# DaehwanKimLab/hisat-genotype

Hardware: NVIDIA B200
Metric: reads typed/sec (higher is better)
Workload: dtype u64 bitsets + f64 EM

## Files before the change

hisat-genotype_b200/csrc/em.cu:

```cuda
#include <cooperative_groups.h>
#include <math.h>
#include <string.h>

#include <algorithm>
#include <vector>

#include "common.cuh"

namespace cg = cooperative_groups;

namespace {

constexpr int EM_THREADS = 1024;
constexpr int EM_WARPS = EM_THREADS / 32;
constexpr int MODE_INIT = 0, MODE_NEXT = 1, MODE_FIRSTK = 2;
constexpr int32_t FK_NONE = 0x7fffffff;

__device__ unsigned long long g_em_trace[16];
__device__ int g_em_trace_on;
struct Trace {
    bool on;
    long long t;
    unsigned long long ns0;
    __device__ __forceinline__ void start() {
        on = g_em_trace_on && blockIdx.x == 0 && threadIdx.x == 0;
        t = on ? clock64() : 0;
        ns0 = 0;
        if (g_em_trace_on && threadIdx.x == 0) asm volatile("mov.u64 %0, %%globaltimer;" : "=l"(ns0));
    }
    __device__ __forceinline__ void finish() {
        if (g_em_trace_on && threadIdx.x == 0) {
            unsigned long long ns1;
            asm volatile("mov.u64 %0, %%globaltimer;" : "=l"(ns1));
            atomicAdd(&g_em_trace[11], ns1 - ns0);
            atomicMax(&g_em_trace[12], ns1 - ns0);
            atomicAdd(&g_em_trace[13], 1ull);
        }
    }
    __device__ __forceinline__ void mark(int k) {
        if (on) {
            const long long n = clock64();
            atomicAdd(&g_em_trace[k], (unsigned long long)(n - t));
            t = n;
        }
    }
    __device__ __forceinline__ void count(int k) {
        if (on) atomicAdd(&g_em_trace[k], 1ull);
    }
};

constexpr int EM_PEER_MAX = 16, EM_PEER_G = 256;
constexpr unsigned long long EM_PEER_TIMEOUT_NS = 4000000000ull;
constexpr size_t EM_PEER_FLAG_BYTES = (size_t)EM_PEER_MAX * EM_PEER_G * 4, EM_PEER_HDR = EM_PEER_FLAG_BYTES + 256;
struct EmPeer {
    int rank, world;
    unsigned char *block[EM_PEER_MAX];
};
__device__ __forceinline__ void st_release_sys(uint32_t *p, uint32_t v) {
    asm volatile("st.release.sys.global.u32 [%0], %1;" ::"l"(p), "r"(v) : "memory");
}
__device__ __forceinline__ uint32_t ld_acquire_sys(const uint32_t *p) {
    uint32_t v;
    asm volatile("ld.acquire.sys.global.u32 %0, [%1];" : "=r"(v) : "l"(p) : "memory");
    return v;
}
__device__ __forceinline__ double ld_sys_f64(const double *p) {
    double v;
    asm volatile("ld.relaxed.sys.global.f64 %0, [%1];" : "=d"(v) : "l"(p) : "memory");
    return v;
}
__device__ __forceinline__ int32_t ld_sys_s32(const int32_t *p) {
    int32_t v;
    asm volatile("ld.relaxed.sys.global.s32 %0, [%1];" : "=r"(v) : "l"(p) : "memory");
    return v;
}

struct EmArgs {
    const uint64_t *bits;
    const double *cnt;
    const double *len;
    int C, A, wp, remove_low, fixed_iters;
    int slab_rows;
    int compact;
    int A_live_max;
    unsigned slab_bytes;
    uint64_t *dense_ws;
    uint64_t *mv_ws;
    int32_t *rep_ws;
    double *mult_ws;
    const unsigned long long *cnt_u64;
    const int32_t *C_ptr;
    const int32_t *class_first;
    int32_t key_offset;
    const EmPeer *peer;
    double *prob;
    uint8_t *in_result;
    int32_t *first_class;
    int32_t *iters_status;
    double *vec;
    uint8_t *live;
    double *part_acc;
    int32_t *part_aux;
    double *red_acc;
    int32_t *red_aux;
};

struct Smem {
    uint64_t *mbar;
    double *red;
    double *p;
    double *w;
    uint8_t *valid;
    uint64_t *slab;
    const int32_t *lv;
    double *cnt;
    uint64_t *cm64;
    unsigned char *c64;
    const int32_t *row_off;
    const int32_t *col_off;
// ... 595 lines not shown
                    }
                    v3[j] = x;
                }
            }
            if (lane == 0) s_flag = flag;
        }
        __syncthreads();
        const int flag = s_flag;
        if (flag == 2) {
            if (tid == 0) *status = HGT_ERR_KEY;
            __syncthreads();
            break;
        }
        if (flag == 1) {
            compact_sweep(a, c, v3, l2, v1, l1, status);
            sweeps += 1;
            last = 3;
        } else {
            last = 0;
        }
        have_last = true;
        if (warp == 0) {
            double d = 0.0;
            for (int j = lane; j < c.n; j += 32)
                if (l0[j]) d += l1[j] ? fabs(v0[j] - v1[j]) : v0[j];
            d = warp_sum(d);
            if (lane == 0) s_diff = d;
        }
        __syncthreads();
        diff = s_diff;
        if (tid < 64) {
            const double t = v0[tid];
            const int tl = l0[tid];
            v0[tid] = v1[tid];
            l0[tid] = l1[tid];
            v1[tid] = t;
            l1[tid] = tl;
        }
        __syncthreads();
        if (last == 0) last = 1;
        if (iter >= 10 && a.remove_low) {
            if (warp == 0) {
                double mx = -1.0;
                for (int j = lane; j < c.n; j += 32)
                    if (l0[j]) mx = fmax(mx, v0[j]);
                mx = warp_max(mx);
                if (mx >= 0.0) {
                    const double thr = mx / 10.0;
                    for (int j = lane; j < c.n; j += 32)
                        if (l0[j] && !(v0[j] >= thr)) {
                            l0[j] = 0;
                            v0[j] = 0.0;
                        }
                }
            }
            __syncthreads();
        }
        iter++;
    }
}

constexpr int DEDUP_CAP = 8192;
constexpr int DEDUP_MAX_LIVE = 6144;
constexpr int DEDUP_COLS = 4;
__host__ __device__ inline bool em_merge_fits(int wp, int A_live_max, size_t slab_bytes) {
    return wp <= DEDUP_COLS * EM_WARPS && A_live_max <= DEDUP_MAX_LIVE && slab_bytes >= (size_t)wp * 64 * 12 + DEDUP_CAP * 4 &&
           slab_bytes >= (size_t)wp * 8 * 32;
}
__host__ __device__ inline bool em_collapse_fits(bool compacted, int C, int wp, int slab_rows) {
    return compacted || (size_t)C * 24 + 64 * 64 <= p_slots((size_t)wp * 64) * 8 + (size_t)slab_rows * 8 + (size_t)slab_rows * wp * 8;
}
__device__ __forceinline__ unsigned long long dedup_mix(unsigned long long x) {
    x ^= x >> 33; x *= 0xff51afd7ed558ccdULL; x ^= x >> 33; x *= 0xc4ceb9fe1a85ec53ULL; x ^= x >> 33;
    return x;
}

__device__ int em_compact_build(const EmArgs &a, Smem &sm, int32_t *lv, int C, int *s_int, bool dedup, Trace &tr) {
    const int tid = threadIdx.x, lane = tid & 31, warp = tid >> 5;
    const int wp = a.wp;
    uint64_t *lw = reinterpret_cast<uint64_t *>(sm.c64);
    int32_t *base = reinterpret_cast<int32_t *>(sm.c64 + 2048);
    for (int j = tid; j < 256; j += EM_THREADS) lw[j] = 0ull;
    __syncthreads();
    {
        uint64_t acc[8];
#pragma unroll
        for (int i = 0; i < 8; i++) acc[i] = 0ull;
        for (int r = warp; r < C; r += EM_WARPS) {
            const uint64_t *row = a.bits + (size_t)r * wp;
#pragma unroll
            for (int i = 0; i < 8; i++) {
                const int j = lane + 32 * i;
                if (j < wp) acc[i] |= row[j];
            }
        }
#pragma unroll
        for (int i = 0; i < 8; i++)
            if (acc[i]) atomicOr(reinterpret_cast<unsigned long long *>(&lw[lane + 32 * i]), (unsigned long long)acc[i]);
    }
    __syncthreads();
    tr.mark(5);
    if (dedup) {
        int32_t *cnt32 = reinterpret_cast<int32_t *>(a.dense_ws);
        const int Atot = wp * 64;
        for (int al = tid; al < Atot; al += EM_THREADS) { cnt32[al] = 0; a.rep_ws[al] = -1; }
        unsigned long long *xs = reinterpret_cast<unsigned long long *>(sm.w);
        uint32_t *ys = reinterpret_cast<uint32_t *>(sm.cnt);
        for (int r = tid; r < C; r += EM_THREADS) {
            const unsigned long long x = dedup_mix((unsigned long long)r + 1ull);
            xs[r] = x;
            ys[r] = (uint32_t)dedup_mix(x ^ 0x9e3779b97f4a7c15ull);
        }
        uint64_t *tile = sm.slab;
        const int T = min(C, (int)(a.slab_bytes / ((size_t)wp * 8)));
        uint64_t pa[DEDUP_COLS], pb[DEDUP_COLS], pc[DEDUP_COLS];
#pragma unroll
        for (int c = 0; c < DEDUP_COLS; c++) pa[c] = pb[c] = pc[c] = 0ull;
        for (int t0 = 0; t0 < C; t0 += T) {
            const int nr = min(T, C - t0);
            __syncthreads();
            {
                const ulonglong2 *src = reinterpret_cast<const ulonglong2 *>(a.bits + (size_t)t0 * wp);
                ulonglong2 *dst = reinterpret_cast<ulonglong2 *>(tile);
                const int n2 = nr * wp / 2;
#pragma unroll 4
                for (int i = tid; i < n2; i += EM_THREADS) dst[i] = __ldg(&src[i]);
            }
            __syncthreads();
            const int j0 = warp * DEDUP_COLS;
            if (j0 < wp) {
                const bool v1 = j0 + 1 < wp, v2 = j0 + 2 < wp, v3 = j0 + 3 < wp;
                for (int r = 0; r < nr; r++) {
                    const ulonglong2 *trow = reinterpret_cast<const ulonglong2 *>(tile + (size_t)r * wp + j0);
                    const ulonglong2 q01 = trow[0], q23 = trow[1];
                    const uint64_t w0 = q01.x, w1 = v1 ? q01.y : 0ull, w2 = v2 ? q23.x : 0ull, w3 = v3 ? q23.y : 0ull;
                    if ((w0 | w1 | w2 | w3) == 0ull) continue;
                    const unsigned long long x = xs[t0 + r];
                    const uint32_t y = ys[t0 + r];
                    const uint64_t m0 = ((x >> lane) & 1ull) ? ~0ull : 0ull, m1 = ((x >> (lane + 32)) & 1ull) ? ~0ull : 0ull,
                                   m2 = ((y >> lane) & 1u) ? ~0ull : 0ull;
                    pa[0] ^= w0 & m0; pb[0] ^= w0 & m1; pc[0] ^= w0 & m2;
                    pa[1] ^= w1 & m0; pb[1] ^= w1 & m1; pc[1] ^= w1 & m2;
                    pa[2] ^= w2 & m0; pb[2] ^= w2 & m1; pc[2] ^= w2 & m2;
                    pa[3] ^= w3 & m0; pb[3] ^= w3 & m1; pc[3] ^= w3 & m2;
                }
            }
        }
        __syncthreads();
        tr.mark(14);
        unsigned long long *sig1 = reinterpret_cast<unsigned long long *>(sm.slab);
        uint32_t *sig2 = reinterpret_cast<uint32_t *>(sig1 + Atot);
#pragma unroll
        for (int c = 0; c < DEDUP_COLS; c++) {
            const int j = warp * DEDUP_COLS + c;
            if (j >= wp) continue;
            const uint64_t live = lw[j];
            for (int b = 0; b < 64; b++) {
                if (!((live >> b) & 1ull)) continue;
                const unsigned m0 = __ballot_sync(0xffffffffu, (pa[c] >> b) & 1ull);
                const unsigned m1 = __ballot_sync(0xffffffffu, (pb[c] >> b) & 1ull);
                const unsigned m2 = __ballot_sync(0xffffffffu, (pc[c] >> b) & 1ull);
                if (lane == 0) {
                    sig1[j * 64 + b] = (unsigned long long)m0 | ((unsigned long long)m1 << 32);
                    sig2[j * 64 + b] = m2;
                }
            }
        }
        __syncthreads();
        uint32_t *occ = sig2 + Atot;
        for (int i = tid; i < DEDUP_CAP; i += EM_THREADS) occ[i] = 0xffffffffu;
        __syncthreads();
        for (int al = tid; al < Atot; al += EM_THREADS) {
            if (!((lw[al >> 6] >> (al & 63)) & 1ull)) continue;
            const unsigned long long h1 = sig1[al];
            const uint32_t h2 = sig2[al];
            unsigned slot = (unsigned)dedup_mix(h1 + h2) & (DEDUP_CAP - 1);
            while (true) {
                const uint32_t prev = atomicCAS(&occ[slot], 0xffffffffu, ((uint32_t)al << 16) | (uint32_t)al);
                if (prev == 0xffffffffu) break;
                const int owner = (int)(prev >> 16);
                if (sig1[owner] == h1 && sig2[owner] == h2) {
                    atomicMin(&occ[slot], ((uint32_t)owner << 16) | (uint32_t)al);
                    break;
                }
                slot = (slot + 1) & (DEDUP_CAP - 1);
            }
            a.rep_ws[al] = (int)slot;
        }
        __syncthreads();
        for (int al = tid; al < Atot; al += EM_THREADS) {
            const int slot = a.rep_ws[al];
            if (slot < 0) continue;
            const int rp = (int)(occ[slot] & 0xffffu);
            a.rep_ws[al] = rp;
            if (rp != al) atomicAdd(&cnt32[rp], 1);
        }
        __syncthreads();
        for (int al = tid; al < Atot; al += EM_THREADS) {
            const int rp = a.rep_ws[al];
            if (rp >= 0 && rp != al) atomicAnd(reinterpret_cast<unsigned long long *>(&lw[al >> 6]), ~(1ull << (al & 63)));
        }
        __syncthreads();
        tr.mark(15);
    }
    if (warp == 0) {
        int run = 0;
        for (int j0 = 0; j0 < wp; j0 += 32) {
            const int j = j0 + lane;
            const int c = j < wp ? __popcll(lw[j]) : 0;
            int incl = c;
#pragma unroll
            for (int o = 1; o < 32; o <<= 1) {
                const int y = __shfl_up_sync(0xffffffffu, incl, o);
                if (lane >= o) incl += y;
            }
            if (j < wp) base[j] = run + incl - c;
            run += __shfl_sync(0xffffffffu, incl, 31);
        }
        if (lane == 0) *s_int = run;
    }
    __syncthreads();
    const int An = *s_int;
    if (An > a.A_live_max) return An;
    for (int j = tid; j < wp; j += EM_THREADS) {
        uint64_t m = lw[j];
        int n = base[j];
        while (m) {
            const int b = __ffsll((long long)m) - 1;
            m &= m - 1;
            lv[n++] = j * 64 + b;
// ... 89 lines not shown
            if (r < C) row_off[r + 1] = run + incl;
            run += __shfl_sync(0xffffffffu, incl, 31);
        }
        if (lane == 0) row_off[0] = 0;
    }
    for (int c = tid; c < wq; c += EM_THREADS) {
        int n = 0;
        for (int w = 0; w < nb; w++) {
            nzpre[(size_t)c * nb + w] = (uint32_t)n;
            n += __popc(nzbits[(size_t)c * nb + w]);
        }
        col_off[c + 1] = n;
    }
    __syncthreads();
    if (warp == 0) {
        int run = 0;
        for (int c0 = 0; c0 < wq; c0 += 32) {
            const int c = c0 + lane;
            const int v = c < wq ? col_off[c + 1] : 0;
            int incl = v;
#pragma unroll
            for (int o = 1; o < 32; o <<= 1) {
                const int y = __shfl_up_sync(0xffffffffu, incl, o);
                if (lane >= o) incl += y;
            }
            if (c < wq) col_off[c + 1] = run + incl;
            run += __shfl_sync(0xffffffffu, incl, 31);
        }
        if (lane == 0) col_off[0] = 0;
    }
    __syncthreads();
    const int nnzw = row_off[C];
    const size_t need = ((fixed + 15) & ~(size_t)15) + (size_t)nnzw * 16 + 32;
    if (need > R_bytes || C > 65535) {
        __syncthreads();
        for (int i = tid; i < C * wpc; i += EM_THREADS) sm.slab[i] = __ldcg(&dense[i]);
        __syncthreads();
        return An;
    }
    uint64_t *r_ent = reinterpret_cast<uint64_t *>(R + ((fixed + 15) & ~(size_t)15));
    uint64_t *c_ent = r_ent + ((nnzw + 1) & ~1);
    for (int r = warp; r < C; r += EM_WARPS) {
        int pos = row_off[r];
        for (int c0 = 0; c0 < wq; c0 += 32) {
            const int c = c0 + lane;
            const uint32_t word = c < wq ? __ldcg(&dense32[(size_t)r * wq + c]) : 0u;
            const unsigned nzm = __ballot_sync(0xffffffffu, word != 0u);
            if (word != 0u) {
                const int e = pos + __popc(nzm & ((1u << lane) - 1u));
                r_ent[e] = (uint64_t)word | ((uint64_t)((uint32_t)c * 264u) << 32);
                const int ce = col_off[c] + (int)nzpre[(size_t)c * nb + (r >> 5)] +
                               __popc(nzbits[(size_t)c * nb + (r >> 5)] & ((1u << (r & 31)) - 1u));
                c_ent[ce] = (uint64_t)word | ((uint64_t)((uint32_t)r * 8u) << 32);
            }
            pos += __popc(nzm);
        }
    }
    __syncthreads();
    sm.row_off = row_off; sm.col_off = col_off;
    sm.r_ent = r_ent; sm.c_ent = c_ent;
    return An;
}

template <int NA, bool COOP>
__global__ void __launch_bounds__(EM_THREADS, 1) em_kernel(const EmArgs *__restrict__ args_arr) {
    extern __shared__ __align__(16) unsigned char smem_raw[];
    EmArgs a = COOP ? args_arr[0] : args_arr[blockIdx.x];
    if (a.C_ptr) a.C = min(*a.C_ptr, a.C);
    const int tid = threadIdx.x;
    const int A_orig = a.A;
    __shared__ int s_status;
    __shared__ int s_int;
    if (tid == 0) s_status = HGT_OK;
    Trace tr, tr_all;
    tr.start();
    tr_all = tr;
    tr.count(10);
    Smem sm;
    sm.mbar = reinterpret_cast<uint64_t *>(smem_raw);
    sm.red = reinterpret_cast<double *>(smem_raw + 16);
    sm.lv = nullptr; sm.cnt = nullptr; sm.cm64 = nullptr; sm.c64 = nullptr;
    sm.row_off = nullptr; sm.col_off = nullptr; sm.r_ent = nullptr; sm.c_ent = nullptr; sm.dense_g = nullptr;
    sm.mult = nullptr;
    bool compacted = false;
    if (!COOP && a.compact) {
        const int wpc_max = max(2, ((a.A_live_max + 63) / 64 + 1) & ~1);
        const size_t Apadc = (size_t)wpc_max * 64, Cpad = (size_t)a.slab_rows;
        unsigned char *q = smem_raw + 16 + 40 * 8;
        sm.c64 = q; q += 4096;
        int32_t *lv = reinterpret_cast<int32_t *>(q); q += Apadc * 4;
        sm.p = reinterpret_cast<double *>(q); q += p_slots(Apadc) * 8;
        sm.w = reinterpret_cast<double *>(q); q += Cpad * 8;
        sm.cnt = reinterpret_cast<double *>(q); q += Cpad * 8;
        sm.cm64 = reinterpret_cast<uint64_t *>(q); q += Cpad * 8;
        sm.slab = reinterpret_cast<uint64_t *>(q); q += a.slab_bytes;
        sm.valid = q;
        for (int al = tid; al < A_orig; al += EM_THREADS) {
            a.prob[al] = 0.0;
            a.in_result[al] = 0;
            a.first_class[al] = FK_NONE;
        }
        const bool dedup = !a.len && a.rep_ws && em_merge_fits(a.wp, a.A_live_max, a.slab_bytes);
        const int An = em_compact_build(a, sm, lv, a.C, &s_int, dedup, tr);
        if (An > a.A_live_max) {
            if (tid == 0) {
                a.iters_status[0] = 0;
                a.iters_status[1] = HGT_ERR_ARG;
                a.iters_status[2] = 0;
            }
            return;
        }
        sm.lv = lv;
        a.A = An;
        a.wp = max(2, ((An + 63) / 64 + 1) & ~1);
        compacted = true;
    } else {
        const int Apad0 = a.wp * 64;
        sm.p = sm.red + 40;
        sm.w = sm.p + p_slots(Apad0);
        sm.slab = reinterpret_cast<uint64_t *>(sm.w + a.slab_rows);
        sm.valid = reinterpret_cast<uint8_t *>(sm.slab + (size_t)a.slab_rows * a.wp);
    }
    const int Apad = a.wp * 64;
    if (tid == 0) {
        mbar_init(sm.mbar, 1);
        fence_barrier_init();
    }
    __syncthreads();
    int row_lo = 0, row_hi = a.C;
    if (COOP) {
        const int G = gridDim.x;
        const int per = (a.C + G - 1) / G;
        row_lo = min(a.C, (int)blockIdx.x * per);
        row_hi = min(a.C, row_lo + per);
    }
    const bool resident = compacted || (row_hi - row_lo) <= a.slab_rows;
    bool loaded = compacted;
    uint32_t parity = 0;
    uint32_t xseq = 0;
    if (COOP && a.peer) xseq = *reinterpret_cast<const volatile uint32_t *>(a.peer->block[a.peer->rank] + EM_PEER_FLAG_BYTES + 4);
    double *v0 = a.vec, *v1 = a.vec + Apad, *v2 = a.vec + 2 * (size_t)Apad, *v3 = a.vec + 3 * (size_t)Apad;
    uint8_t *l0 = a.live, *l1 = a.live + Apad, *l2 = a.live + 2 * (size_t)Apad;
    tr.mark(5);
    em_sweep<NA, COOP>(a, sm, MODE_INIT, nullptr, nullptr, v0, l0, nullptr, row_lo, row_hi, resident, loaded,
                       parity, &s_status, tr, xseq);
    double diff = 1.0;
    int iter = 0, sweeps = 0;
    const double *last_in = v0;
    const uint8_t *last_live = l0;
    bool have_last = false;
    const bool compact_ok = !COOP && em_collapse_fits(compacted, a.C, a.wp, a.slab_rows);
    while (a.fixed_iters > 0 ? iter < a.fixed_iters : (diff > 0.0001 && iter < 1000)) {
        if (s_status != HGT_OK) break;
        if (compact_ok && (iter == 0 || (iter > 10 && a.remove_low))) {
            int cnt_live = 0;
            for (int al = tid; al < a.A; al += EM_THREADS)
                if (l0[al]) cnt_live += (sm.mult && sm.mult[al] != 1.0) ? 1000 : 1;
            cnt_live = (int)block_sum((double)cnt_live, sm.red);
            if (cnt_live > 0 && cnt_live <= 64) {
                Compact c;
                unsigned char *base = compacted ? sm.c64 : reinterpret_cast<unsigned char *>(sm.p);
                c.v = reinterpret_cast<double *>(base);
                c.len = c.v + 256;
                c.q = c.len + 64;
                c.lv = reinterpret_cast<int *>(c.q + 64);
                c.l = c.lv + 64;
                if (compacted) {
                    c.cnt = sm.cnt;
                    c.w = sm.w;
                    c.cm = sm.cm64;
                } else {
                    c.cnt = reinterpret_cast<double *>(c.l + 192);
                    c.w = c.cnt + a.C;
                    c.cm = reinterpret_cast<uint64_t *>(c.w + a.C);
                }
                c.n = cnt_live;
                __syncthreads();
                if (tid < 32) {
                    int n = 0;
                    for (int a0 = 0; a0 < a.A; a0 += 32) {
                        const int al = a0 + tid;
                        const bool k = al < a.A && l0[al];
                        const unsigned m = __ballot_sync(0xffffffffu, k);
                        if (k) c.lv[n + __popc(m & ((1u << tid) - 1u))] = al;
                        n += __popc(m);
                    }
                }
                __syncthreads();
                if (tid < 64) {
                    const bool k = tid < c.n;
                    const int al = k ? c.lv[tid] : 0;
                    c.v[tid] = k ? v0[al] : 0.0;
                    c.v[64 + tid] = c.v[128 + tid] = c.v[192 + tid] = 0.0;
                    c.l[tid] = k ? 1 : 0;
                    c.l[64 + tid] = c.l[128 + tid] = 0;
                    c.len[tid] = (k && a.len) ? a.len[orig_allele(sm, al)] : 1.0;
                }
                {
                    const int lane = tid & 31, warp = tid >> 5;
                    const int a_lo = lane < c.n ? c.lv[lane] : -1, a_hi = lane + 32 < c.n ? c.lv[lane + 32] : -1;
                    for (int r = warp; r < a.C; r += EM_WARPS) {
                        const uint64_t *row = (compacted ? sm.dense_g : a.bits) + (size_t)r * a.wp;
                        const bool b_lo = a_lo >= 0 && ((__ldcg(&row[a_lo >> 6]) >> (a_lo & 63)) & 1ull);
                        const bool b_hi = a_hi >= 0 && ((__ldcg(&row[a_hi >> 6]) >> (a_hi & 63)) & 1ull);
                        const unsigned m_lo = __ballot_sync(0xffffffffu, b_lo), m_hi = __ballot_sync(0xffffffffu, b_hi);
                        if (lane == 0) {
                            c.cm[r] = (uint64_t)m_lo | ((uint64_t)m_hi << 32);
                            if (!compacted) c.cnt[r] = a.cnt_u64 ? (double)a.cnt_u64[r] : a.cnt[r];
                        }
                    }
                }
// ... 58 lines not shown
            __syncthreads();
            break;
        }
        if (ssv > 0.0) {
            const double g = -sqrt(ssr / ssv);
            for (int al = tid; al < a.A; al += EM_THREADS) {
                double x = 0.0;
                if (l0[al]) {
                    const double r = v1[al] - v0[al];
                    const double v = v2[al] - v1[al] - r;
                    x = v0[al] - 2 * g * r + g * g * v;
                    x = x > 0.0 ? x : 0.0;
                }
                v3[al] = x;
            }
            __syncthreads();
            tr.mark(6);
            em_sweep<NA, COOP>(a, sm, MODE_NEXT, v3, l2, v1, l1, nullptr, row_lo, row_hi, resident, loaded,
                               parity, &s_status, tr, xseq);
            sweeps += 1;
            last_in = v3;
            last_live = l2;
        } else {
            last_in = v0;
            last_live = l0;
        }
        have_last = true;
        double d = 0.0;
        for (int al = tid; al < a.A; al += EM_THREADS)
            if (l0[al]) d += l1[al] ? fabs(v0[al] - v1[al]) : v0[al];
        diff = block_sum(d, sm.red);
        {
            double *tv = v0; v0 = v1; v1 = tv;
            uint8_t *tl = l0; l0 = l1; l1 = tl;
        }
        if (iter >= 10 && a.remove_low) {
            em_prune(a, sm, v0, l0);
        }
        iter++;
    }
    if (s_status == HGT_OK) {
        if (a.remove_low) em_prune(a, sm, v0, l0);
        double part = 0.0;
        int nk = 0;
        for (int al = tid; al < a.A; al += EM_THREADS)
            if (l0[al]) {
                part += a.len ? v0[al] / a.len[orig_allele(sm, al)] : v0[al];
                nk = 1;
            }
        const double total = block_sum(part, sm.red);
        if (block_or(nk) && !(total > 0.0) && !(total < 0.0)) {
            if (tid == 0) s_status = HGT_ERR_ZERODIV;
            __syncthreads();
        }
        const bool writer = !COOP || blockIdx.x == 0;
        if (writer) {
            for (int al = tid; al < a.A; al += EM_THREADS) {
                const bool key = l0[al];
                const int ao = orig_allele(sm, al);
                a.prob[ao] = key ? (a.len ? v0[al] / a.len[ao] / total : (sm.mult ? v0[al] / sm.mult[al] / total : v0[al] / total)) : 0.0;
                a.in_result[ao] = key ? 1 : 0;
            }
        }
        if (have_last) {
            em_sweep<NA, COOP>(a, sm, MODE_FIRSTK, last_in, last_live, nullptr, nullptr, a.first_class, row_lo,
                               row_hi, resident, loaded, parity, &s_status, tr, xseq);
        } else if (writer) {
            for (int al = tid; al < A_orig; al += EM_THREADS) a.first_class[al] = FK_NONE;
        }
        if (sm.mult) {
            __syncthreads();
            for (int al = tid; al < A_orig; al += EM_THREADS) {
                const int rp = a.rep_ws[al];
                if (rp >= 0 && rp != al) {
                    a.prob[al] = a.prob[rp];
                    a.in_result[al] = a.in_result[rp];
                    a.first_class[al] = a.first_class[rp];
                }
            }
        }
    }
    tr.mark(6);
    tr_all.mark(8);
    tr_all.finish();
    if (tid == 0 && (!COOP || blockIdx.x == 0)) {
        a.iters_status[0] = iter;
        a.iters_status[1] = s_status;
        a.iters_status[2] = sweeps;
        if (COOP && a.peer) *reinterpret_cast<uint32_t *>(a.peer->block[a.peer->rank] + EM_PEER_FLAG_BYTES + 4) = xseq;
    }
}

template <int NA>
__global__ void __launch_bounds__(EM_THREADS, 1) em_part_kernel(EmArgs a, int mode, const double *__restrict__ pin) {
    extern __shared__ __align__(16) unsigned char smem_raw[];
    const int tid = threadIdx.x;
    Smem sm;
    sm.mbar = reinterpret_cast<uint64_t *>(smem_raw);
    sm.red = reinterpret_cast<double *>(smem_raw + 16);
    sm.lv = nullptr; sm.cnt = nullptr; sm.cm64 = nullptr; sm.c64 = nullptr;
    sm.row_off = nullptr; sm.col_off = nullptr; sm.r_ent = nullptr; sm.c_ent = nullptr; sm.dense_g = nullptr;
    sm.mult = nullptr;
    const int Apad = a.wp * 64;
    sm.p = sm.red + 40;
    sm.w = sm.p + p_slots(Apad);
    sm.slab = reinterpret_cast<uint64_t *>(sm.w + a.slab_rows);
    sm.valid = reinterpret_cast<uint8_t *>(sm.slab + (size_t)a.slab_rows * a.wp);
    if (tid == 0) {
        mbar_init(sm.mbar, 1);
        fence_barrier_init();
    }
    __syncthreads();
    const int G = gridDim.x, g = blockIdx.x;
    const int per = (a.C + G - 1) / G;
    const int row_lo = min(a.C, g * per), row_hi = min(a.C, row_lo + per);
    bool loaded = false;
    uint32_t parity = 0;
    double acc[NA];
    int32_t fk[NA];
    uint32_t hit = 0;
    Trace tr;
    tr.on = false; tr.t = 0; tr.ns0 = 0;
    em_accumulate<NA>(a, sm, mode, pin, nullptr, row_lo, row_hi, false, loaded, parity, acc, fk, hit, tr);
#pragma unroll
    for (int i = 0; i < NA; i++) {
        const int al = tid + i * EM_THREADS;
        if (al < a.A) {
            a.part_acc[(size_t)g * Apad + al] = acc[i];
            a.part_aux[(size_t)g * Apad + al] = (mode == MODE_FIRSTK) ? fk[i] : (int32_t)((hit >> i) & 1u);
        }
    }
}

__global__ void em_part_reduce_kernel(int G, int A, int Apad, int mode, const double *__restrict__ part_acc,
                                      const int32_t *__restrict__ part_aux, double *__restrict__ acc_out,
                                      int32_t *__restrict__ aux_out, double *__restrict__ hit_out) {
    const int al = blockIdx.x * blockDim.x + threadIdx.x;
    if (al >= A) return;
    double s = 0.0;
    int32_t x = (mode == MODE_FIRSTK) ? FK_NONE : 0;
    for (int g = 0; g < G; g++) {
        s += part_acc[(size_t)g * Apad + al];
        const int32_t y = part_aux[(size_t)g * Apad + al];
        x = (mode == MODE_FIRSTK) ? min(x, y) : (x | y);
    }
    if (acc_out) acc_out[al] = s;
    if (aux_out) aux_out[al] = x;
    if (hit_out) hit_out[al] = (double)x;
}

struct EmPlan {
    int na;
    int slab_rows;
    size_t smem;
};

int em_plan(const hgt_ctx *ctx, int rows_per_cta, int A, int wp, EmPlan *plan) {
    const int Apad = wp * 64;
    if (A > 16 * EM_THREADS) {
        hgt_set_error("EM kernel supports at most %d alleles per problem (got %d)", 16 * EM_THREADS, A);
        return HGT_ERR_UNSUPPORTED;
    }
    int na = 1;
    while (na * EM_THREADS < Apad) na *= 2;
    const size_t fixed = 16 + 40 * 8 + p_slots(Apad) * 8;
    const size_t budget = ctx->smem_optin > 1024 ? ctx->smem_optin - 1024 : 0;
    if (fixed + 2 * ((size_t)wp * 8 + 9) > budget) {
        hgt_set_error("EM kernel: %d alleles do not fit shared memory", A);
        return HGT_ERR_UNSUPPORTED;
    }
    size_t rows = (budget - fixed) / ((size_t)wp * 8 + 9);
    rows &= ~(size_t)1;
    int want = rows_per_cta < 2 ? 2 : ((rows_per_cta + 1) & ~1);
    if ((size_t)want < rows) rows = want;
    plan->na = na;
    plan->slab_rows = (int)rows;
    plan->smem = fixed + rows * ((size_t)wp * 8 + 8) + rows + 16;
    return HGT_OK;
}

template <bool COOP>
int em_launch(hgt_ctx *ctx, cudaStream_t st, const EmArgs *d_args, int grid, int na, size_t smem) {
    void (*kern)(const EmArgs *) = nullptr;
    switch (na) {
        case 1: kern = em_kernel<1, COOP>; break;
        case 2: kern = em_kernel<2, COOP>; break;
        case 4: kern = em_kernel<4, COOP>; break;
        case 8: kern = em_kernel<8, COOP>; break;
        default: kern = em_kernel<16, COOP>; break;
    }
    HGT_CUDA(hgt_smem_at_least((const void *)kern, smem));
    if (COOP) {
        void *params[] = {(void *)&d_args};
        HGT_CUDA(cudaLaunchCooperativeKernel((void *)kern, dim3(grid), dim3(EM_THREADS), params, smem, st));
    } else {
        kern<<<grid, EM_THREADS, smem, st>>>(d_args);
        HGT_CUDA(cudaGetLastError());
    }
    ctx->launches++;
    return HGT_OK;
}

constexpr size_t EM_DENSE_SCRATCH = 232448;
struct EmShape {
    int C, A, wp, A_live_max;
};
int em_plan_batched(const hgt_ctx *ctx, const EmShape &sh, EmArgs *a, int *na, size_t *smem) {
    const size_t budget = ctx->smem_optin > 1024 ? ctx->smem_optin - 1024 : 0;
    int alive = sh.A_live_max < sh.A ? sh.A_live_max : sh.A;
    if (alive < 1) alive = 1;
    const int wpc = hgt_row_pitch(alive);
    const size_t Apadc = (size_t)wpc * 64;
    const size_t Cpad = sh.C < 2 ? 2 : (size_t)((sh.C + 1) & ~1);
    const size_t dense = Cpad * (size_t)wpc * 8;
    const size_t other = 16 + 40 * 8 + 4096 + Apadc * 4 + p_slots(Apadc) * 8 + Cpad * 25 + 16;
    size_t need = other + dense;
    if (sh.wp <= 256 && need <= budget && dense <= EM_DENSE_SCRATCH && Apadc <= (size_t)16 * EM_THREADS) {
        const size_t nb = (Cpad + 31) / 32;
        size_t want = 4 * dense + (Cpad + 1 + 2 * (size_t)wpc + 1 + 4 * (size_t)wpc * nb) * 4 + 64;
        want = (want + 15) & ~(size_t)15;
        size_t slab = dense;
        if (other + want <= budget) slab = want;
        else if (budget - other > dense) slab = (budget - other) & ~(size_t)15;
        need = other + slab;
        a->slab_bytes = (unsigned)slab;
        a->compact = 1;
        a->A_live_max = alive;
        a->slab_rows = (int)Cpad;
        int n = 1;
        while ((size_t)n * EM_THREADS < Apadc) n *= 2;
        *na = n;
        *smem = need;
        return HGT_OK;
    }
    EmPlan plan;
    HGT_CHECK(em_plan(ctx, sh.C < 1 ? 1 : sh.C, sh.A, sh.wp, &plan));
    a->compact = 0;
    a->slab_bytes = 0;
    a->A_live_max = sh.A;
    a->slab_rows = plan.slab_rows;
    *na = plan.na;
    *smem = plan.smem;
    return HGT_OK;
}

int em_launch_batched(hgt_ctx *ctx, cudaStream_t st, int n, const EmArgs *planned, const int *na, const size_t *smem,
                      EmArgs *h_args, EmArgs *d_args, bool h_pinned) {
    std::vector<int> order(n);
    for (int i = 0; i < n; i++) order[i] = i;
    std::stable_sort(order.begin(), order.end(), [&](int x, int y) {
        if (planned[x].compact != planned[y].compact) return planned[x].compact < planned[y].compact;
        return (double)planned[x].C * planned[x].A_live_max > (double)planned[y].C * planned[y].A_live_max;
    });
    for (int i = 0; i < n; i++) h_args[i] = planned[order[i]];
    if (h_pinned) HGT_CUDA(hgt_small_h2d(d_args, h_args, (size_t)n * sizeof(EmArgs), st));
    else HGT_CUDA(cudaMemcpyAsync(d_args, h_args, (size_t)n * sizeof(EmArgs), cudaMemcpyHostToDevice, st));
    int na_max = 1;
    size_t sm = 0;
    for (int i = 0; i < n; i++) {
        if (na[i] > na_max) na_max = na[i];
        if (smem[i] > sm) sm = smem[i];
    }
    HGT_CHECK(em_launch<false>(ctx, st, d_args, n, na_max, sm));
    return HGT_OK;
}

inline size_t align_up(size_t x, size_t a) { return (x + a - 1) / a * a; }
inline size_t em_compact_scratch_bytes(int wp) { return align_up(EM_DENSE_SCRATCH + (size_t)wp * 48 + (size_t)wp * 64 * 12, 256); }
inline void em_set_scratch(EmArgs *a, void *scratch) {
    unsigned char *b = static_cast<unsigned char *>(scratch);
    a->dense_ws = reinterpret_cast<uint64_t *>(b);
    a->mv_ws = reinterpret_cast<uint64_t *>(b + EM_DENSE_SCRATCH);
    a->mult_ws = reinterpret_cast<double *>(b + EM_DENSE_SCRATCH + (size_t)a->wp * 48);
    a->rep_ws = reinterpret_cast<int32_t *>(b + EM_DENSE_SCRATCH + (size_t)a->wp * 48 + (size_t)a->wp * 64 * 8);
}

struct EmWs {
    EmArgs *d_args;
    double *vec;
    uint8_t *live;
    double *part_acc;
    int32_t *part_aux;
    double *red_acc;
    int32_t *red_aux;
    void *scratch;
};
size_t em_ws_bytes(int sm_count, int A) {
    const size_t Apad = (size_t)hgt_row_pitch(A) * 64;
    size_t b = 512;
    b += align_up(4 * Apad * 8, 256);
    b += align_up(4 * Apad, 256);
    b += align_up((size_t)sm_count * Apad * 8, 256);
    b += align_up((size_t)sm_count * Apad * 4, 256);
    b += align_up(Apad * 8, 256) + align_up(Apad * 4, 256);
    b += em_compact_scratch_bytes(hgt_row_pitch(A));
    return b;
}
EmWs em_ws_carve(void *ws, int sm_count, int A) {
    const size_t Apad = (size_t)hgt_row_pitch(A) * 64;
    unsigned char *p = static_cast<unsigned char *>(ws);
    EmWs w;
    w.d_args = reinterpret_cast<EmArgs *>(p); p += 512;
    w.vec = reinterpret_cast<double *>(p); p += align_up(4 * Apad * 8, 256);
    w.live = p; p += align_up(4 * Apad, 256);
    w.part_acc = reinterpret_cast<double *>(p); p += align_up((size_t)sm_count * Apad * 8, 256);
    w.part_aux = reinterpret_cast<int32_t *>(p); p += align_up((size_t)sm_count * Apad * 4, 256);
    w.red_acc = reinterpret_cast<double *>(p); p += align_up(Apad * 8, 256);
    w.red_aux = reinterpret_cast<int32_t *>(p); p += align_up(Apad * 4, 256);
    w.scratch = p;
    return w;
}

int em_dev_plan(const hgt_ctx *ctx, int n_classes, int n_alleles, int wp, int n_ctas, int A_live_max, EmArgs *a,
                EmPlan *plan, int *grid) {
    int G = n_ctas;
    if (G <= 0) {
        const size_t bytes = (size_t)n_classes * wp * 8;
        G = bytes <= 160 * 1024 ? 1 : ctx->sm_count;
    }
    if (G > ctx->sm_count) G = ctx->sm_count;
    if (G > n_classes) G = n_classes;
    if (G < 1) G = 1;
    if (G == 1) {
        const EmShape sh{n_classes, n_alleles, wp, A_live_max};
        int na = 1;
        size_t smem = 0;
        HGT_CHECK(em_plan_batched(ctx, sh, a, &na, &smem));
        plan->na = na; plan->smem = smem; plan->slab_rows = a->slab_rows;
    } else {
        HGT_CHECK(em_plan(ctx, (n_classes + G - 1) / G, n_alleles, wp, plan));
        a->compact = 0; a->A_live_max = n_alleles; a->slab_bytes = 0;
        a->slab_rows = plan->slab_rows;
    }
    *grid = G;
    return HGT_OK;
// ... 462 lines not shown
        for (int al = tid; al < A; al += EM_THREADS) {
            const double a0 = p0[al], an = pn[al];
            const uint8_t k0 = l0[al], kn = ln[al];
            if (k0) d += kn ? fabs(a0 - an) : a0;
            lastp[al] = use3 ? (l2[al] ? p3[al] : 0.0) : (k0 ? a0 : 0.0);
            lastl[al] = use3 ? l2[al] : k0;
            p0[al] = an;
            l0[al] = kn;
        }
        d = block_sum(d, red);
        if (it >= 10 && remove_low) shard_prune(A, p0, l0, red);
        if (tid == 0) s.scal[4] = d;
    } else {
        double *p0 = s.vec, *prob = s.vec + A;
        uint8_t *l0 = s.live;
        if (remove_low) shard_prune(A, p0, l0, red);
        double part = 0.0;
        int any = 0;
        for (int al = tid; al < A; al += EM_THREADS)
            if (l0[al]) {
                part += len ? p0[al] / len[al] : p0[al];
                any = 1;
            }
        const double total = block_sum(part, red);
        any = block_or(any);
        if (any && !(total > 0.0) && !(total < 0.0) && tid == 0) s.scal[3] = 1.0;
        for (int al = tid; al < A; al += EM_THREADS)
            prob[al] = l0[al] ? (len ? p0[al] / len[al] / total : p0[al] / total) : 0.0;
        if (tid == 0) s.scal[6] = any ? 1.0 : 0.0;
    }
}

extern "C" size_t hgt_em_shard_state_bytes(int32_t n_alleles) {
    const size_t A = (size_t)(n_alleles < 1 ? 1 : n_alleles);
    return align_up((8 * A + 8) * 8 + ((A + 1) & ~(size_t)1) * 4 + 5 * A, 256);
}

extern "C" int hgt_em_shard_sweep_dev(hgt_ctx *ctx, void *stream, const uint64_t *class_bits, const double *class_count_f64,
                                      const uint64_t *class_count_u64, const int32_t *class_key, int32_t key_offset,
                                      int32_t n_classes, int32_t n_alleles, int32_t wp, int32_t mode, int32_t src,
                                      void *state, void *workspace) {
    if (!state || src > 5) {
        hgt_set_error("hgt_em_shard_sweep_dev: bad argument");
        return HGT_ERR_ARG;
    }
    const ShardState s = shard_state(state, n_alleles);
    const double *pin = (mode == MODE_INIT || src < 0) ? nullptr : s.vec + (size_t)src * n_alleles;
    if (mode == MODE_FIRSTK)
        return em_partial_impl(ctx, stream, class_bits, class_count_f64, class_count_u64, class_key, key_offset, n_classes,
                               n_alleles, wp, pin, mode, nullptr, s.fk, nullptr, workspace);
    return em_partial_impl(ctx, stream, class_bits, class_count_f64, class_count_u64, class_key, key_offset, n_classes,
                           n_alleles, wp, pin, mode, s.red, nullptr, s.red + n_alleles, workspace);
}

extern "C" int hgt_em_shard_vec_dev(hgt_ctx *ctx, void *stream, int32_t op, int32_t n_alleles, void *state,
                                    const double *allele_len, int32_t src, int32_t dst, int32_t iteration,
                                    int32_t remove_low) {
    if (!ctx || !state || op < SHARD_FINISH || op > SHARD_FINAL || n_alleles < 1 || n_alleles > 16 * EM_THREADS ||
        (op == SHARD_FINISH && (src > 3 || dst < 0 || dst > 4 || dst == 3))) {
        hgt_set_error("hgt_em_shard_vec_dev: bad argument");
        return HGT_ERR_ARG;
    }
    em_shard_vec_kernel<<<1, EM_THREADS, 0, static_cast<cudaStream_t>(stream)>>>(op, n_alleles, state, allele_len, src, dst,
                                                                                 iteration, remove_low);
    HGT_CUDA(cudaGetLastError());
    ctx->launches++;
    return HGT_OK;
}

#include "em_internal.h"

size_t hgt_em_problem_ws_bytes(int wp) {
    const size_t Apad = (size_t)wp * 64;
    return align_up(4 * Apad * 8 + 4 * Apad, 256) + em_compact_scratch_bytes(wp);
}
extern "C" int hgt_em_trace(hgt_ctx *ctx, int32_t enable, uint64_t *cycles16) {
    if (!ctx) return HGT_ERR_ARG;
    HGT_CUDA(cudaSetDevice(ctx->device));
    HGT_CUDA(cudaDeviceSynchronize());
    unsigned long long z[16];
    if (cycles16) {
        HGT_CUDA(cudaMemcpyFromSymbol(z, g_em_trace, sizeof(z)));
        for (int i = 0; i < 16; i++) cycles16[i] = z[i];
    }
    memset(z, 0, sizeof(z));
    HGT_CUDA(cudaMemcpyToSymbol(g_em_trace, z, sizeof(z)));
    const int on = enable ? 1 : 0;
    HGT_CUDA(cudaMemcpyToSymbol(g_em_trace_on, &on, sizeof(on)));
    return HGT_OK;
}

size_t hgt_em_args_bytes(int n_problems) { return align_up((size_t)n_problems * sizeof(EmArgs), 256); }

bool hgt_em_wants_coop(const hgt_ctx *ctx, int C, int A, int wp, int A_live_max, int n_problems) {
    EmArgs a;
    int na = 1;
    size_t smem = 0;
    const EmShape sh{C < 1 ? 1 : C, A, wp, A_live_max};
    if (em_plan_batched(ctx, sh, &a, &na, &smem) != HGT_OK) return false;
    if (a.compact || C < 2) return false;
    const size_t bytes = (size_t)C * wp * 8;
    return bytes > ((size_t)4 << 20) || (n_problems <= 6 && bytes > ((size_t)256 << 10));
}
size_t hgt_em_coop_ws_bytes(const hgt_ctx *ctx, int A) { return em_ws_bytes(ctx->sm_count, A); }

extern "C" int hgt_em_form(const hgt_ctx *ctx, int32_t n_classes, int32_t n_alleles, int32_t wp, int32_t has_lengths,
                           int32_t n_ctas, int32_t a_live_max, int32_t n_problems, hgt_em_form_info *out) {
    if (!ctx || !out || n_classes < 1 || n_alleles < 1 || wp < hgt_row_pitch(n_alleles) || (wp & 1)) {
        hgt_set_error("hgt_em_form: need a context, an output, n_classes >= 1, n_alleles >= 1 and an even wp >= "
                      "hgt_row_pitch(n_alleles)");
        return HGT_ERR_ARG;
    }
    if (a_live_max < 1 || a_live_max > n_alleles) a_live_max = n_alleles;
    EmArgs a;
    EmPlan plan;
    int G = 1;
    HGT_CHECK(em_dev_plan(ctx, n_classes, n_alleles, wp, n_ctas, a_live_max, &a, &plan, &G));
    out->form = G > 1 ? HGT_EM_FORM_COOP : (a.compact ? HGT_EM_FORM_COMPACT : HGT_EM_FORM_STREAM);
    out->grid = G;
    out->na = plan.na;
    out->slab_rows = plan.slab_rows;
    out->slab_bytes = a.slab_bytes;
    out->merge = a.compact && !has_lengths && em_merge_fits(wp, a.A_live_max, a.slab_bytes);
    out->collapse = G == 1 && em_collapse_fits(a.compact, n_classes, wp, plan.slab_rows);
    out->batch_coop = hgt_em_wants_coop(ctx, n_classes, n_alleles, wp, a_live_max, n_problems);
    return HGT_OK;
}

int hgt_em_batch_dev(hgt_ctx *ctx, cudaStream_t st, int n_problems, const EmDevProblem *pr, void *h_args, void *d_args) {
    if (n_problems <= 0) return HGT_OK;
    std::vector<EmArgs> args, coop;
    std::vector<int> nas, coop_na, coop_g;
    std::vector<size_t> smems, coop_smem;
    for (int i = 0; i < n_problems; i++) {
        EmArgs a;
        const size_t Apad = (size_t)pr[i].wp * 64;
        a.bits = pr[i].bits; a.cnt = nullptr; a.len = pr[i].len;
        a.C = pr[i].C_max; a.A = pr[i].A; a.wp = pr[i].wp; a.remove_low = pr[i].remove_low; a.fixed_iters = 0;
        a.cnt_u64 = pr[i].cnt; a.C_ptr = pr[i].C_ptr; a.class_first = pr[i].class_first; a.key_offset = 0; a.peer = nullptr;
        a.prob = pr[i].prob; a.in_result = pr[i].in_result; a.first_class = pr[i].first_class;
        a.iters_status = pr[i].iters_status;
        a.part_acc = nullptr; a.part_aux = nullptr; a.red_acc = nullptr; a.red_aux = nullptr;
        if (pr[i].coop_ws && pr[i].C_max > 1) {
            int G = ctx->sm_count;
            if (G > pr[i].C_max) G = pr[i].C_max;
            EmPlan plan;
            HGT_CHECK(em_plan(ctx, (pr[i].C_max + G - 1) / G, pr[i].A, pr[i].wp, &plan));
            EmWs w = em_ws_carve(pr[i].coop_ws, ctx->sm_count, pr[i].A);
            a.vec = w.vec; a.live = w.live; a.part_acc = w.part_acc; a.part_aux = w.part_aux;
            a.red_acc = w.red_acc; a.red_aux = w.red_aux;
            em_set_scratch(&a, w.scratch);
            a.compact = 0; a.A_live_max = pr[i].A; a.slab_bytes = 0;
            a.slab_rows = plan.slab_rows;
            coop.push_back(a);
            coop_na.push_back(plan.na);
            coop_smem.push_back(plan.smem);
            coop_g.push_back(G);
            continue;
        }
        const EmShape sh{pr[i].C_max < 1 ? 1 : pr[i].C_max, pr[i].A, pr[i].wp, pr[i].A_live_max};
        int na = 1;
        size_t smem = 0;
        HGT_CHECK(em_plan_batched(ctx, sh, &a, &na, &smem));
        a.vec = static_cast<double *>(pr[i].ws);
        a.live = reinterpret_cast<uint8_t *>(a.vec + 4 * Apad);
        em_set_scratch(&a, static_cast<unsigned char *>(pr[i].ws) + align_up(4 * Apad * 8 + 4 * Apad, 256));
        args.push_back(a);
        nas.push_back(na);
        smems.push_back(smem);
// ... 12 lines not shown
```

Measured before the change: 84.78 million.

## Use TMA bulk copies for dedup tiles and fold live-word OR into dedup pass

In the dedup compaction path, the cooperative per-thread global-to-shared tile copy is replaced by a single bulk async copy tracked by an mbarrier. The separate pass that ORs all rows to find live allele words is skipped and computed inside the dedup loop instead. Mbarrier init moves earlier so it is ready for this use. The batched launcher also sorts problems that have length arrays separately, and per-CTA trace recording is added for diagnostics. The risks are mbarrier parity misuse across tiles and bulk-copy alignment requirements on the tile size.

```diff
diff --git a/hisat-genotype_b200/csrc/em.cu b/hisat-genotype_b200/csrc/em.cu
--- a/hisat-genotype_b200/csrc/em.cu
+++ b/hisat-genotype_b200/csrc/em.cu
@@ -1,5 +1,6 @@
 #include <cooperative_groups.h>
 #include <math.h>
+#include <stdlib.h>
 #include <string.h>
 
 #include <algorithm>
@@ -18,6 +19,13 @@
 
 __device__ unsigned long long g_em_trace[16];
 __device__ int g_em_trace_on;
+constexpr int EM_TRACE_CTAS = 16384;
+struct EmCtaRec {
+    unsigned long long t0, t1;
+    int32_t grid, cta, C, A_live_max, wp, has_len, An, wq, nnzw, sweeps;
+};
+__device__ EmCtaRec g_em_cta[EM_TRACE_CTAS];
+__device__ unsigned int g_em_cta_n;
 struct Trace {
     bool on;
     long long t;
@@ -28,13 +36,18 @@
         ns0 = 0;
         if (g_em_trace_on && threadIdx.x == 0) asm volatile("mov.u64 %0, %%globaltimer;" : "=l"(ns0));
     }
-    __device__ __forceinline__ void finish() {
+    template <typename Args>
+    __device__ __forceinline__ void finish(const Args *host, int An, int wq, int nnzw, int sweeps) {
         if (g_em_trace_on && threadIdx.x == 0) {
             unsigned long long ns1;
             asm volatile("mov.u64 %0, %%globaltimer;" : "=l"(ns1));
             atomicAdd(&g_em_trace[11], ns1 - ns0);
             atomicMax(&g_em_trace[12], ns1 - ns0);
             atomicAdd(&g_em_trace[13], 1ull);
+            const unsigned k = atomicAdd(&g_em_cta_n, 1u);
+            if (k < EM_TRACE_CTAS)
+                g_em_cta[k] = EmCtaRec{ns0, ns1, (int32_t)gridDim.x, (int32_t)blockIdx.x, host->C, host->A_live_max, host->wp,
+                                       host->len ? 1 : 0, An, wq, nnzw, sweeps};
         }
     }
     __device__ __forceinline__ void mark(int k) {
@@ -796,7 +809,7 @@
     int32_t *base = reinterpret_cast<int32_t *>(sm.c64 + 2048);
     for (int j = tid; j < 256; j += EM_THREADS) lw[j] = 0ull;
     __syncthreads();
-    {
+    if (!dedup) {
         uint64_t acc[8];
 #pragma unroll
         for (int i = 0; i < 8; i++) acc[i] = 0ull;
@@ -830,18 +843,20 @@
         uint64_t pa[DEDUP_COLS], pb[DEDUP_COLS], pc[DEDUP_COLS];
 #pragma unroll
         for (int c = 0; c < DEDUP_COLS; c++) pa[c] = pb[c] = pc[c] = 0ull;
+        const int j0 = warp * DEDUP_COLS;
+        uint64_t orw = 0ull;
+        uint32_t parity = 0;
         for (int t0 = 0; t0 < C; t0 += T) {
             const int nr = min(T, C - t0);
+            fence_proxy_async();
             __syncthreads();
-            {
-                const ulonglong2 *src = reinterpret_cast<const ulonglong2 *>(a.bits + (size_t)t0 * wp);
-                ulonglong2 *dst = reinterpret_cast<ulonglong2 *>(tile);
-                const int n2 = nr * wp / 2;
-#pragma unroll 4
-                for (int i = tid; i < n2; i += EM_THREADS) dst[i] = __ldg(&src[i]);
-            }
-            __syncthreads();
-            const int j0 = warp * DEDUP_COLS;
+            if (tid == 0) {
+                const uint32_t bytes = (uint32_t)nr * (uint32_t)wp * 8u;
+                mbar_expect_tx(sm.mbar, bytes);
+                bulk_g2s(tile, a.bits + (size_t)t0 * wp, bytes, sm.mbar);
+            }
+            mbar_wait(sm.mbar, parity);
+            parity ^= 1u;
             if (j0 < wp) {
                 const bool v1 = j0 + 1 < wp, v2 = j0 + 2 < wp, v3 = j0 + 3 < wp;
                 for (int r = 0; r < nr; r++) {
@@ -849,6 +864,7 @@
                     const ulonglong2 q01 = trow[0], q23 = trow[1];
                     const uint64_t w0 = q01.x, w1 = v1 ? q01.y : 0ull, w2 = v2 ? q23.x : 0ull, w3 = v3 ? q23.y : 0ull;
                     if ((w0 | w1 | w2 | w3) == 0ull) continue;
+                    orw |= lane == 0 ? w0 : lane == 1 ? w1 : lane == 2 ? w2 : w3;
                     const unsigned long long x = xs[t0 + r];
                     const uint32_t y = ys[t0 + r];
                     const uint64_t m0 = ((x >> lane) & 1ull) ? ~0ull : 0ull, m1 = ((x >> (lane + 32)) & 1ull) ? ~0ull : 0ull,
@@ -860,6 +876,7 @@
                 }
             }
         }
+        if (lane < DEDUP_COLS && j0 + lane < wp) lw[j0 + lane] = orw;
         __syncthreads();
         tr.mark(14);
         unsigned long long *sig1 = reinterpret_cast<unsigned long long *>(sm.slab);
@@ -1115,6 +1132,11 @@
     sm.lv = nullptr; sm.cnt = nullptr; sm.cm64 = nullptr; sm.c64 = nullptr;
     sm.row_off = nullptr; sm.col_off = nullptr; sm.r_ent = nullptr; sm.c_ent = nullptr; sm.dense_g = nullptr;
     sm.mult = nullptr;
+    if (tid == 0) {
+        mbar_init(sm.mbar, 1);
+        fence_barrier_init();
+    }
+    __syncthreads();
     bool compacted = false;
     if (!COOP && a.compact) {
         const int wpc_max = max(2, ((a.A_live_max + 63) / 64 + 1) & ~1);
@@ -1155,11 +1177,6 @@
         sm.valid = reinterpret_cast<uint8_t *>(sm.slab + (size_t)a.slab_rows * a.wp);
     }
     const int Apad = a.wp * 64;
-    if (tid == 0) {
-        mbar_init(sm.mbar, 1);
-        fence_barrier_init();
-    }
-    __syncthreads();
     int row_lo = 0, row_hi = a.C;
     if (COOP) {
         const int G = gridDim.x;
@@ -1384,7 +1401,8 @@
     }
     tr.mark(6);
     tr_all.mark(8);
-    tr_all.finish();
+    tr_all.finish(args_arr + (COOP ? 0 : blockIdx.x), compacted ? a.A : -1, compacted ? 2 * a.wp : -1,
+                  sm.row_off ? sm.row_off[a.C] : -1, sweeps);
     if (tid == 0 && (!COOP || blockIdx.x == 0)) {
         a.iters_status[0] = iter;
         a.iters_status[1] = s_status;
@@ -1551,8 +1569,12 @@
     std::vector<int> order(n);
     for (int i = 0; i < n; i++) order[i] = i;
     std::stable_sort(order.begin(), order.end(), [&](int x, int y) {
-        if (planned[x].compact != planned[y].compact) return planned[x].compact < planned[y].compact;
-        return (double)planned[x].C * planned[x].A_live_max > (double)planned[y].C * planned[y].A_live_max;
+        const EmArgs &p = planned[x], &q = planned[y];
+        if (p.compact != q.compact) return p.compact < q.compact;
+        const bool pl = p.len != nullptr, ql = q.len != nullptr;
+        if (pl != ql) return pl < ql;
+        if (pl) return p.A_live_max != q.A_live_max ? p.A_live_max > q.A_live_max : p.C > q.C;
+        return (double)p.C * p.A_live_max > (double)q.C * q.A_live_max;
     });
     for (int i = 0; i < n; i++) h_args[i] = planned[order[i]];
     if (h_pinned) HGT_CUDA(hgt_small_h2d(d_args, h_args, (size_t)n * sizeof(EmArgs), st));
@@ -2181,9 +2203,29 @@
     if (cycles16) {
         HGT_CUDA(cudaMemcpyFromSymbol(z, g_em_trace, sizeof(z)));
         for (int i = 0; i < 16; i++) cycles16[i] = z[i];
+        const char *path = getenv("HGT_EM_TRACE_CTAS");
+        if (path && *path) {
+            unsigned n = 0;
+            HGT_CUDA(cudaMemcpyFromSymbol(&n, g_em_cta_n, sizeof(n)));
+            n = std::min(n, (unsigned)EM_TRACE_CTAS);
+            std::vector<EmCtaRec> rec(n);
+            if (n) HGT_CUDA(cudaMemcpyFromSymbol(rec.data(), g_em_cta, n * sizeof(EmCtaRec)));
+            FILE *f = fopen(path, "a");
+            if (!f) {
+                hgt_set_error("hgt_em_trace: cannot write %s", path);
+                return HGT_ERR_ARG;
+            }
+            if (ftell(f) == 0) fprintf(f, "t0_ns,t1_ns,grid,cta,C,A_live_max,wp,has_len,A_compact,word_cols,nnz_words,sweeps\n");
+            for (const EmCtaRec &r : rec)
+                fprintf(f, "%llu,%llu,%d,%d,%d,%d,%d,%d,%d,%d,%d,%d\n", r.t0, r.t1, r.grid, r.cta, r.C, r.A_live_max, r.wp,
+                        r.has_len, r.An, r.wq, r.nnzw, r.sweeps);
+            fclose(f);
+        }
     }
     memset(z, 0, sizeof(z));
     HGT_CUDA(cudaMemcpyToSymbol(g_em_trace, z, sizeof(z)));
+    const unsigned n0 = 0;
+    HGT_CUDA(cudaMemcpyToSymbol(g_em_cta_n, &n0, sizeof(n0)));
     const int on = enable ? 1 : 0;
     HGT_CUDA(cudaMemcpyToSymbol(g_em_trace_on, &on, sizeof(on)));
     return HGT_OK;
```

After: 86.13 million (median of 6 runs). 1.02x the previous value.
